# okieraised/rs-face-detection-tflite

Measured on AMD Instinct MI355X. Metric: faces/sec at batch=256 (256x256 back-camera) per GPU, higher is better.
Workload: dtype f32

## Files before the change

rs-face-detection-tflite_amd/csrc/engine.cpp:

```cpp
#include "engine.hpp"
#include "launch.hpp"

#include <algorithm>
#include <cstdio>
#include <cstdlib>
#include <cstring>
#include <stdexcept>

namespace mi {

void hip_check(hipError_t e, const char* what) {
    if (e != hipSuccess) throw std::runtime_error(std::string(what) + ": " + hipGetErrorString(e));
}

namespace {
template <class T>
void upload(T*& dev, std::vector<T>& host, const char* what_alloc, const char* what_copy) {
    if (dev) hip_check(hipFree(dev), "hipFree");
    dev = nullptr;
    if (host.empty()) return;
    hip_check(hipMalloc(reinterpret_cast<void**>(&dev), host.size() * sizeof(T)), what_alloc);
    hip_check(hipMemcpy(dev, host.data(), host.size() * sizeof(T), hipMemcpyHostToDevice), what_copy);
    std::vector<T>().swap(host);
}
// ... 53 lines not shown

const Model::Option* Model::find_option(const std::string& key) {
    using O = Option;
    constexpr int kMax = 0x7fffffff;
    static const Option table[] = {
        {"chunk", &Model::chunk_, 0, kMax, 0},
        {"graph", &Model::use_graph_, 0, 1, 0},
        {"fuse", &Model::fuse_level_, 0, 5, O::kReplan},
        {"res_budget", &Model::res_budget_, 16, 156, O::kReplan | O::kKiB},
        {"pipe", &Model::pipe_max_, 0, 4, O::kReplan},
        {"small_chain", &Model::small_chain_, 0, 64, O::kFreeSmall},
        {"pipe_rows", &Model::pipe_rows_, 1 << 1 | 1 << 2 | 1 << 4, 0, O::kOneOf},
        {"pipe_band", &Model::pipe_band_, 0, 4096, 0},
        {"strip", &Model::strip_, 0, 1, 0},
        {"stem_fuse", &Model::stem_fuse_, 0, 1, 0},
        {"stem_mfma", &Model::stem_mfma_, 0, 2, O::kForms},
        {"conv_mfma", &Model::conv_mfma_, 0, 1, 0},
        {"conv_bf16", &Model::conv_bf16_, 0, 2, O::kReplan},
        {"stem_run", &Model::stem_run_, 0, 32, 0},
        {"pair_fuse", &Model::pair_fuse_, 0, 1, 0},
        {"mdb_band", &Model::mdb_band_, 0, 4096, 0},
        {"chain_fixed", &Model::chain_fixed_, 0, 1, 0},
        {"chain_sched", &Model::chain_sched_, 0, 1, 0},
        {"mchain", &Model::mchain_, 0, 1, 0},
        {"tail", &Model::tail_, 0, 1, O::kReplan},
        {"tail_pre", &Model::tail_pre_, 0, 2, 0},
        {"tail_g", &Model::tail_g_, 0, 64, 0},
        {"band", &Model::band_, 0, 2, O::kReplan},
        {"band_test_fail", &Model::band_test_fail_, 0, 1, O::kWriteOnly},
        {"band_test_absent", &Model::band_test_absent_, 0, 256, O::kWriteOnly},
        {"band_test_gen", nullptr, 0, kMax, O::kBandGen | O::kWriteOnly},
        {"band_wide", &Model::band_wide_ok_, 0, 1, O::kReplan},
        {"band_fork", &Model::band_fork_, 0, 1, O::kReplan},
        {"band_nw", &Model::band_nw_, 8, 256, O::kReplan},
        {"band_fail_streak", &Model::band_fail_streak_, 0, 0, O::kReadOnly},
        {"band_wraps", &Model::band_wraps_, 0, 0, O::kReadOnly},
        {"fork", &Model::fork_, 0, 1, 0},
        {"heads", &Model::head_streams_opt_, 1, kHeadStreams, O::kReplan},
        {"reuse", &Model::reuse_, 0, 1, O::kReplan},
        {"lanes", &Model::lanes_, 1, 4, 0},
        {"test_poison", &Model::test_poison_, 1 << 1 | 1 << 2, 0, O::kOneOf | O::kKeepGraphs},
    };
    for (const Option& o : table)
        if (key == o.key) return &o;
    return nullptr;
}

void Model::set_option(const std::string& key, int value) {
    const Option* o = find_option(key);
    if (!o || (o->flags & Option::kReadOnly)) throw std::runtime_error("unknown option '" + key + "'");
    int v = (o->lo == 0 && o->hi == 1) ? value != 0 : std::min(o->hi, std::max(o->lo, value));
    if (o->flags & Option::kOneOf) v = (value >= 0 && value < 31 && (o->lo >> value & 1)) ? value : 0;
    if (o->flags & Option::kForms) v = (value >= o->lo && value <= o->hi) ? value : 1;
    if (o->flags & Option::kKiB) v *= 1024;
    if (o->flags & Option::kBandGen) { band_gen_ = static_cast<unsigned>(v); band_gen_force_ = true; }
    else this->*o->field = v;
    if (o->flags & Option::kKeepGraphs) return;
    if (o->flags & Option::kReplan) dirty_ = true;
    if ((o->flags & Option::kFreeSmall) && d_small_) { hipFree(d_small_); d_small_ = nullptr; small_floats_ = 0; }
    invalidate_graphs();
    chunk_cap_ = 0;
}

int Model::get_option(const std::string& key) const {
    const Option* o = find_option(key);
    if (!o || (o->flags & Option::kWriteOnly)) throw std::runtime_error("unknown option '" + key + "'");
    const int v = this->*o->field;
    return (o->flags & Option::kKiB) ? v / 1024 : v;
}

void Model::rebuild() {
    if (d_small_) { hipFree(d_small_); d_small_ = nullptr; small_floats_ = 0; }
    hip_check(hipSetDevice(device_), "hipSetDevice");
    invalidate_graphs();
    plan_ = build_plan(parse_tflite(blob_.data(), blob_.size()), fuse_level_, pipe_max_, res_budget_, tail_ != 0);
    if (!reuse_) {
        long off = 0;
        for (size_t t = 0; t < plan_.graph.tensors.size(); t++)
            if (plan_.root_offset[t] >= 0) { plan_.root_offset[t] = off; off += plan_.root_elems[t]; }
// ... 154 lines not shown
        st.bytes += bytes;
        st.macs += macs;
        auto dims = [](const std::vector<int>& sh) {
            std::string d;
            for (size_t q = 1; q < sh.size(); q++) d += (q > 1 ? "x" : "") + std::to_string(sh[q]);
            return d;
        };
        if (static_cast<int>(i) == first.launches[k].node) st.detail = dims(si) + "->";
        st.detail = st.detail.substr(0, st.detail.find("->") + 2) + dims(so);
    }
    return stats;
}

LaunchCtx Model::launch_ctx(const float* in, int chunk_start, int frames) const {
    LaunchCtx c;
    c.weights = d_weights_;
    c.arena = d_arena_ + static_cast<size_t>(plan_.arena_floats_per_frame) * chunk_cap_ * arena_lane_;
    c.in = in; c.out = d_out_.data();
    c.small = d_small_; c.small_floats = small_floats_;
    c.progs = d_programs_; c.tail_progs = d_tail_programs_;
    c.band_prog = d_band_prog_; c.band_consts = d_band_consts_; c.band_ws = d_band_ws_; c.band_sync = d_band_sync_; c.band_fail = d_band_fail_;
    c.chunk_cap = chunk_cap_; c.chunk_start = chunk_start; c.F = frames;
    c.u8_frames = u8_.frames; c.u8_lut = u8_.lut; c.u8_frame_bytes = u8_.frame_bytes; c.u8_row_bytes = u8_.row_bytes;
    c.strip = strip_; c.pair_fuse = pair_fuse_; c.stem_fuse = stem_fuse_; c.stem_mfma = stem_mfma_; c.stem_run = stem_run_; c.mchain = mchain_; c.conv_mfma = conv_mfma_; c.conv_bf16 = conv_bf16_;
    c.small_chain = small_chain_; c.lanes = lanes_;
    c.pipe_rows = pipe_rows_; c.pipe_band = pipe_band_; c.mdb_band = mdb_band_; c.tail_pre = tail_pre_; c.tail_g = tail_g_;
    c.fork = fork_ && lanes_ == 1;
    c.cu_count = device_cu_count();
    c.band = band_use_ && chunk_start == 0;
    c.band_test_absent = band_test_absent_;
    return c;
}

namespace {
int issue(const Launch& l, hipStream_t s, int chain_fixed, int chain_sched) {
    auto many = [&](int (*f)(const BlockArgs*, int, void*)) { return f(l.blocks.data(), static_cast<int>(l.blocks.size()), s); };
    switch (l.to) {
        case Launcher::Conv: return launch_conv(std::get<ConvArgs>(l.args), s);
        case Launcher::HeadGemm: return launch_head_gemm(std::get<HeadGemmArgs>(l.args), s);
        case Launcher::Dw: return launch_dw(std::get<DwArgs>(l.args), s);
        case Launcher::Xc: return launch_xc(std::get<XcArgs>(l.args), s);
        case Launcher::Mdblock: return launch_mdblock(std::get<DblockArgs>(l.args), s);
        case Launcher::Dblock: return launch_dblock(std::get<DblockArgs>(l.args), s);
        case Launcher::Mbneck: return launch_mbneck(std::get<BneckArgs>(l.args), s);
        case Launcher::Bneck: return launch_bneck(std::get<BneckArgs>(l.args), s);
        case Launcher::Tail: return launch_tail(std::get<TailLaunch>(l.args), s);
        case Launcher::Resident: return launch_resident(std::get<ResLaunch>(l.args), s);
        case Launcher::Chain: return launch_chain(std::get<ChainArgs>(l.args), s, chain_fixed, chain_sched);
        case Launcher::StripPipe: return many(launch_strip_pipe);
        case Launcher::MstripChain: return many(launch_mstrip_chain);
        case Launcher::SmallChain: {
            int rc = 0;
            for (size_t k = 0; k < l.blocks.size() && rc == 0; k++) rc = l.blocks[k].sh == 1 ? launch_strip(l.blocks[k], s) : launch_block(l.blocks[k], s);
            return rc;
        }
        case Launcher::Ms2: return launch_ms2(std::get<BlockArgs>(l.args), s);
        case Launcher::Mwalk: return launch_mwalk(std::get<BlockArgs>(l.args), s);
        case Launcher::Strip: return launch_strip(std::get<BlockArgs>(l.args), s);
        case Launcher::Mstrip: return launch_mstrip(std::get<BlockArgs>(l.args), s);
        case Launcher::Block: return launch_block(std::get<BlockArgs>(l.args), s);
        case Launcher::Add: return launch_add(std::get<EltArgs>(l.args), s);
        case Launcher::Act: return launch_act(std::get<EltArgs>(l.args), s);
        case Launcher::Maxpool: return launch_maxpool(std::get<EltArgs>(l.args), s);
        case Launcher::Padc: return launch_padc(std::get<EltArgs>(l.args), s);
        case Launcher::Resize2x: return launch_resize2x(std::get<EltArgs>(l.args), s);
        case Launcher::DepthToSpace: return launch_depth_to_space(std::get<EltArgs>(l.args), s);
        case Launcher::Bandnet: return launch_bandnet(std::get<BandLaunch>(l.args), s);
        case Launcher::Avgpool: return launch_avgpool(std::get<EltArgs>(l.args), s);
        case Launcher::L2norm: return launch_l2norm_rows(std::get<EltArgs>(l.args), s);
        case Launcher::Transpose: return launch_transpose(std::get<EltArgs>(l.args), s);
    }
    return 0;
}
// ... 228 lines not shown
            in_stage_floats_ = need;
        }
        hip_check(hipMemcpyAsync(d_in_stage_, in, need * sizeof(float), hipMemcpyHostToDevice, s), "H2D input");
        if (test_poison_ && in_stage_floats_ > need)
            hip_check(hipMemsetAsync(d_in_stage_ + need, test_poison_ == 1 ? 0xFF : 0x7F, (in_stage_floats_ - need) * sizeof(float), s), "hipMemsetAsync poison stage");
        din = d_in_stage_;
    }
    run_device(din, batch, s);
    for (int k = 0; k < num_outputs(); k++) {
        if (!outs[k]) continue;
        hip_check(hipMemcpyAsync(outs[k], d_out_[k], output_elems(k) * sizeof(float) * batch,
                                 mem == 0 ? hipMemcpyDeviceToHost : hipMemcpyDeviceToDevice, s), "copy outputs");
    }
    if (mem == 0 || !stream) hip_check(hipStreamSynchronize(s), "hipStreamSynchronize");
}

size_t Model::debug_tensor(int tensor, int frame, float* dst, size_t cap) {
    const Graph& g = plan_.graph;
    if (tensor < 0 || tensor >= static_cast<int>(g.tensors.size())) throw std::runtime_error("tensor index out of range");
    if (frame < 0 || frame >= last_chunk_frames_) throw std::runtime_error("frame outside the last chunk");
    bool produced = false;
    for (const Node& n : plan_.nodes) produced |= (n.out == tensor);
    if (!produced) throw std::runtime_error("tensor was fused away (or is an input/constant)");
    long fs;
    float* p = tensor_ptr_mut(plan_, launch_ctx(nullptr, 0, last_chunk_frames_), tensor, &fs);
    size_t n = std::min(cap, g.tensors[tensor].elems());
    hip_check(hipDeviceSynchronize(), "sync");
    hip_check(hipMemcpy(dst, p + static_cast<long>(frame) * fs, n * sizeof(float), hipMemcpyDeviceToHost), "D2H debug");
    return n;
}

}
```

rs-face-detection-tflite_amd/csrc/engine.hpp:

```cpp
#pragma once

#include <hip/hip_runtime.h>

#include <map>
#include <memory>
#include <string>
#include <vector>

#include "bandplan.hpp"
#include "consts.hpp"
#include "launches.hpp"
#include "plan.hpp"

namespace mi {

void hip_check(hipError_t e, const char* what);

class Model {
   public:
    Model(const uint8_t* bytes, size_t n, int device);
    ~Model();
    Model(const Model&) = delete;
    Model& operator=(const Model&) = delete;

// ... 30 lines not shown
    struct Option;
    static const Option* find_option(const std::string& key);
    void build_bandnet();
    void free_bandnet();
    bool band_usable(int batch) const;
    void band_before_launch(hipStream_t s);
    void poison_scratch(hipStream_t s);
    void ensure_capacity(int batch);
    LaunchCtx launch_ctx(const float* in, int chunk_start, int frames) const;
    void enqueue_chunk(const float* in, int chunk_start, int frames, hipStream_t s, std::vector<hipEvent_t>* marks = nullptr, Lowered* keep = nullptr);
    void enqueue_all(const float* in, int batch, hipStream_t s);
    void invalidate_graphs();

    int device_ = 0;
    std::vector<uint8_t> blob_;
    Plan plan_;
    int fuse_level_ = 5, pipe_max_ = 4, tail_ = 1, reuse_ = 1;
    int res_budget_ = 156 * 1024;
    int chunk_ = 0, lanes_ = 1, use_graph_ = 1;
    int fork_ = 1, head_streams_opt_ = 1;
    int conv_mfma_ = 1;
    int conv_bf16_ = 0;
    int strip_ = 1, stem_fuse_ = 1, stem_mfma_ = 1, stem_run_ = 0, pair_fuse_ = 1, mchain_ = 1, chain_fixed_ = 1, chain_sched_ = 1;
    int pipe_rows_ = 0, pipe_band_ = 0, mdb_band_ = 0;
    int tail_pre_ = 0, tail_g_ = 0;
    int arena_lane_ = 0;
    std::vector<hipStream_t> side_streams_;
    std::vector<hipEvent_t> lane_events_;
    SideSchedule sched_;
    std::vector<hipStream_t> head_streams_;
    std::vector<hipEvent_t> head_events_;
    bool dirty_ = true;

    float* d_weights_ = nullptr;
    PlanConsts consts_;
    int profile_inner_ = 1;

    ResStage* d_programs_ = nullptr;
    TailStage* d_tail_programs_ = nullptr;
    float* d_arena_ = nullptr;
    size_t arena_floats_ = 0;
    int chunk_cap_ = 0;
    int batch_cap_ = 0;
    std::vector<float*> d_out_;
    float* d_in_stage_ = nullptr;
    size_t in_stage_floats_ = 0;
// ... 54 lines not shown
```

rs-face-detection-tflite_amd/csrc/kernels.hpp:

```cpp
#pragma once

#include <cstddef>
#include <cstdint>

namespace mi {

enum ActKind : int { ACT_NONE = 0, ACT_RELU = 1, ACT_RELU6 = 2, ACT_PRELU = 3 };
enum ResMode : int { RES_NONE = 0, RES_DIRECT = 1, RES_MAXPOOL = 2, RES_UP2X = 3 };

struct Epilogue {
    const float* bias = nullptr;
    const float* alpha = nullptr;
    const float* res = nullptr;
    long res_fs = 0;
    int res_mode = RES_NONE;
    int res_C = 0;
    int res_W = 0, res_H = 0;
    int act = ACT_NONE;
    int res_after = 0;
};

struct ConvArgs {
    const float* in = nullptr;
    const uint8_t* in_u8 = nullptr;
// ... 254 lines not shown
int strip_consts_floats(int C);
void strip_pack_consts(int C, const float* w_dw, const float* b_dw, const float* w_pw, const float* bias, const float* alpha, int act, float* dst);
const char* strip_kernel_label(const BlockArgs& a, char* buf, size_t cap);
int launch_mwalk(const BlockArgs& a, void* stream);
bool mwalk_kernel_supports(const BlockArgs& a);
bool mwalk_shape_ok(int W, int C, int Co);
int mwalk_consts_floats(int W, int C, int Co);
void mwalk_pack_consts(int W, int C, int Co, const float* w_dw, const float* b_dw, const float* w_pw, const float* bias, const float* alpha, int act, float* dst);
const char* mwalk_kernel_label(const BlockArgs& a, char* buf, size_t cap);
int launch_ms2(const BlockArgs& a, void* stream);
bool ms2_kernel_supports(const BlockArgs& a);
bool ms2_shape_ok(int W, int C, int Co, bool skip);
int ms2_consts_floats(int W, int C, int Co, bool skip);
void ms2_pack_consts(int W, int C, int Co, bool skip, const float* w_dw, const float* b_dw, const float* w_pw, const float* bias, const float* alpha, int act, float* dst);
const char* ms2_kernel_label(const BlockArgs& a, char* buf, size_t cap);
int launch_mstrip(const BlockArgs& a, void* stream);
bool mstrip_kernel_supports(const BlockArgs& a);
bool mstrip_shape_ok(int C, int Co);
int mstrip_consts_floats(int C);
void mstrip_pack_consts(int C, const float* w_dw, const float* b_dw, const float* w_pw, const float* bias, const float* alpha, int act, float* dst);
const char* mstrip_kernel_label(const BlockArgs& a, char* buf, size_t cap);
bool mstrip_chain_supports(const BlockArgs* blocks, int n);
int launch_mstrip_chain(const BlockArgs* blocks, int n, void* stream);
bool strip_pipe_supports(const BlockArgs* blocks, int n);
bool strip_pipe_shape_ok(int C, int W);
bool strip_tail_shape_ok(int C, int Co, int H, int W);
int strip_consts_s2_floats(int C, int Co);
void strip_pack_consts_s2(int C, int Co, const float* w_dw, const float* b_dw, const float* w_pw, const float* bias, const float* alpha, int act, float* dst);
int launch_strip_pipe(const BlockArgs* blocks, int n, void* stream);
const char* strip_pipe_label(const BlockArgs* blocks, int n, char* buf, size_t cap);
int strip_pipe_rows_per_step(int H, int hint = 0);
int launch_chain(const ChainArgs& a, void* stream, int fixed = 1, int sched = 1);

struct BneckBlock {
    const float* w1 = nullptr;
    const float* w2 = nullptr;
    const float* consts = nullptr;
    float hi1 = 0.f, hi2 = 0.f;
    const float* mconsts = nullptr;
    int act1 = ACT_RELU, act2 = ACT_RELU;
};
constexpr int kMaxBneck = 6;
struct BneckArgs {
    const float* in = nullptr;
    float* out = nullptr;
    long in_fs = 0, out_fs = 0;
// ... 163 lines not shown
```

rs-face-detection-tflite_amd/csrc/launches.cpp:

```cpp
#include "launches.hpp"

#include <algorithm>
#include <cmath>
#include <cstdio>
#include <cstdlib>
#include <stdexcept>

namespace mi {

namespace {
void same_pad(int in, int k, int stride, int out, int* before) { *before = std::max(0, (out - 1) * stride + k - in) / 2; }
bool is_view(const Node& n) { return n.kind == Node::Reshape || n.kind == Node::Concat; }
int dim(const std::vector<int>& v, size_t d) { return d < v.size() ? v[d] : 1; }
float clamp_of(int act) { return act == ACT_RELU6 ? 6.f : INFINITY; }
}

bool band_cut(const BandPlan& bp, size_t i) { return static_cast<int>(i) >= bp.first && !bp.node_runs[i]; }

int band_run_launches(const Plan& plan, const BandPlan& bp) {
    int launches = 1;
    for (size_t i = 0; i < plan.nodes.size(); i++)
        if (!is_view(plan.nodes[i]) && !band_cut(bp, i)) launches++;
    return launches;
}
// ... 519 lines not shown
                if (b.ep.res_mode != RES_NONE) { b.ep.res = cur; b.ep.res_fs = cur_fs; }
                if (k == nb - 1) { b.out = op; b.out_fs = out_fs; } else { b.out = T[k & 1]; b.out_fs = fsz; }
                ok = b.sh == 1 ? strip_kernel_supports(b) : block_kernel_supports(b);
                cur = b.out; cur_fs = b.out_fs;
            }
            if (ok) {
                l.to = Launcher::SmallChain;
                if (want_labels) {
                    char name[48];
                    const bool s2 = sb[static_cast<size_t>(nb - 1)].sh == 2;
                    snprintf(buf, sizeof buf, "%s x%d%s (small batch)", strip_kernel_label(sb[0], name, sizeof name), s2 ? nb - 1 : nb, s2 ? " + block_kernel" : "");
                    l.label = buf;
                }
                l.blocks = std::move(sb);
                return;
            }
        }
        if (!strip_pipe_supports(blk.data(), static_cast<int>(blk.size()))) throw std::runtime_error("chain node without a kernel");
        l.to = Launcher::StripPipe;
        if (want_labels) l.label = strip_pipe_label(blk.data(), static_cast<int>(blk.size()), buf, sizeof buf);
        l.blocks = std::move(blk);
    }

    size_t block(size_t i, Launch& l) const {
        const Node& n = plan.nodes[i];
        const BlockArgs a = block_args(i);
        char buf[96];
        if (c.strip && c.pair_fuse && pc.node_pair[i] >= 0 && i + 1 < plan.nodes.size() && !sched.event_after[i] && sched.slot[i + 1] < 0 && sched.slot[i] < 0) {
            const Node& nb = plan.nodes[i + 1];
            const DblockArgs d = dblock_args(a.in, a.in_fs, n.in[0], nb.out, n, nb, pc.node_pair[i], true);
            const bool apart = d.out + d.out_fs * c.F <= d.in || d.in + d.in_fs * c.F <= d.out;
            if (apart && mdblock_kernel_supports(d)) {
                set(l, Launcher::Mdblock, d, lab("mdblock_kernel<pair>"));
                return 2;
            }
        }
        if (c.strip && ms2_kernel_supports(a)) {
            set(l, Launcher::Ms2, a, want_labels ? ms2_kernel_label(a, buf, sizeof buf) : nullptr);
            return 1;
        }
        if (c.strip && mwalk_kernel_supports(a)) {
            set(l, Launcher::Mwalk, a, want_labels ? mwalk_kernel_label(a, buf, sizeof buf) : nullptr);
            return 1;
        }
        const bool strip = c.strip && strip_kernel_supports(a);
        const bool mstrip = c.strip && !strip && mstrip_kernel_supports(a);
        if (mstrip && c.mchain && c.lanes == 1) {
            std::vector<BlockArgs> run{a};
            for (size_t j = i + 1; j < plan.nodes.size() && run.size() < 8; j++) {
                const Node& m = plan.nodes[j];
                if (m.kind != Node::Block || m.w < 0 || m.in.size() != 1 || m.in[0] != plan.nodes[j - 1].out || pc.node_strip[j] < 0 || sched.slot[j] >= 0) break;
                if (shape(m.in[0]).size() != 4 || shape(m.out) != shape(m.in[0]) || m.ept >= 0) break;
                if (m.res >= 0 && (m.res != m.in[0] || m.res_mode != RES_DIRECT || m.res_after)) break;
                run.push_back(block_args(j));
                if (!mstrip_chain_supports(run.data(), static_cast<int>(run.size()))) { run.pop_back(); break; }
            }
            if (run.size() >= 2) {
                l.to = Launcher::MstripChain;
                if (want_labels) { snprintf(buf, sizeof buf, "mstrip_chain_kernel<%d,%d>", a.C / 4, a.ep.act == ACT_RELU ? 1 : 0); l.label = buf; }
                l.blocks = std::move(run);
                return l.blocks.size();
            }
        }
        if (strip) set(l, Launcher::Strip, a, want_labels ? strip_kernel_label(a, buf, sizeof buf) : nullptr);
        else if (mstrip) set(l, Launcher::Mstrip, a, want_labels ? mstrip_kernel_label(a, buf, sizeof buf) : nullptr);
        else set(l, Launcher::Block, a, want_labels ? block_kernel_label(a, buf, sizeof buf) : nullptr);
        return 1;
    }
};

}

Lowered lower_chunk(const Plan& plan, const PlanConsts& consts, const BandPlan& bp, const SideSchedule& sched, const LaunchCtx& c, bool want_labels) {
    const Lowering lo{plan, consts, bp, sched, c, want_labels};
    const size_t N = plan.nodes.size();
    Lowered out;
// ... 37 lines not shown
```

rs-face-detection-tflite_amd/csrc/launches.hpp:

```cpp
#pragma once

#include <string>
#include <variant>
#include <vector>

#include "bandplan.hpp"
#include "consts.hpp"
#include "kernels.hpp"
#include "plan.hpp"

namespace mi {

constexpr int kHeadStreams = 4;

struct SideSchedule {
    std::vector<int> slot, wait;
    std::vector<char> event_after;
};
SideSchedule schedule_side_streams(const Plan& plan, int head_streams);

struct LaunchCtx {
    const float* weights = nullptr;
    float* arena = nullptr;
    const float* in = nullptr;
    float* const* out = nullptr;
    float* small = nullptr;
    size_t small_floats = 0;
    const ResStage* progs = nullptr;
    const TailStage* tail_progs = nullptr;
    const BandPacked* band_prog = nullptr;
    const float* band_consts = nullptr;
    float* band_ws = nullptr;
    unsigned* band_sync = nullptr;
    int* band_fail = nullptr;
    int chunk_cap = 0, chunk_start = 0, F = 0;
    const uint8_t* u8_frames = nullptr;
    const float* u8_lut = nullptr;
    long u8_frame_bytes = 0;
    int u8_row_bytes = 0;
    int strip = 1, pair_fuse = 1, stem_fuse = 1, stem_mfma = 1, stem_run = 0, mchain = 1, small_chain = 16, lanes = 1;
    int conv_mfma = 1;
    int conv_bf16 = 0;
    int pipe_rows = 0, pipe_band = 0, mdb_band = 0, tail_pre = 0, tail_g = 0;
    bool fork = true;
    int cu_count = 256;
    bool band = false;
    int band_test_absent = 0;
};

enum class Launcher {
    Conv, HeadGemm, Dw, Xc, Mdblock, Dblock, Mbneck, Bneck, Tail, Resident, Chain, StripPipe, SmallChain, Ms2, Mwalk, MstripChain, Strip, Mstrip, Block,
    Add, Act, Maxpool, Padc, Resize2x, DepthToSpace, Bandnet, Avgpool, L2norm, Transpose
};

struct Launch {
    Launcher to = Launcher::Conv;
    std::variant<ConvArgs, HeadGemmArgs, DwArgs, XcArgs, DblockArgs, BneckArgs, TailLaunch, ResLaunch, ChainArgs, BlockArgs, EltArgs, BandLaunch> args;
    std::vector<BlockArgs> blocks;
    int node = -1, last = -1;
    int slot = -1;
    int wait = -1;
    bool record = false;
    std::string label;
};

struct Lowered {
    std::vector<Launch> launches;
    std::vector<int> launch_of_node;
};
Lowered lower_chunk(const Plan& plan, const PlanConsts& consts, const BandPlan& band_plan, const SideSchedule& sched, const LaunchCtx& ctx, bool want_labels);

float* tensor_ptr_mut(const Plan& plan, const LaunchCtx& ctx, int t, long* frame_stride);

bool band_cut(const BandPlan& band_plan, size_t i);
int band_run_launches(const Plan& plan, const BandPlan& band_plan);
// ... 5 lines not shown
```

rs-face-detection-tflite_amd/csrc/mrow.hpp:

```cpp
#pragma once

#include <hip/hip_runtime.h>

#include <type_traits>
#include <utility>

#include "kernels.hpp"
#include "launch.hpp"
#include "wave_sync.hpp"

namespace mi {

namespace {

typedef float df32x4 __attribute__((ext_vector_type(4)));

__device__ __forceinline__ void dwg_barrier() {
    asm volatile("s_waitcnt lgkmcnt(0)\n\ts_barrier" ::: "memory");
}

template <class F, int... KS>
__device__ __forceinline__ void dfor_each(F&& f, std::integer_sequence<int, KS...>) { (f(std::integral_constant<int, KS>{}), ...); }

typedef float dv2f __attribute__((ext_vector_type(2)));
// ... 102 lines not shown
            aC[ks].s[0] = c;
            aPN[ks].s[0] = n;
            asm volatile("" : "+v"(aC[ks].s[0]), "+v"(aPN[ks].s[0]));
            pch[nt] = pc;
        }
        if constexpr (EMIT) {
            if constexpr (NP > 0) __builtin_amdgcn_sched_barrier(0);
#pragma unroll
            for (int mt = 0; mt < MT; mt++)
#pragma unroll
                for (int nt = 0; nt < WT; nt++) D[mt][nt] = __builtin_amdgcn_mfma_f32_16x16x4f32(aw[mt], pch[nt], D[mt][nt], 0, 0, 0);
        }
        asm volatile("s_waitcnt lgkmcnt(0)" ::: "memory");
        if constexpr (ks + 1 < CK) landed(xs[(ks + 1) & 1], av[(ks + 1) & 1]);
        __builtin_amdgcn_sched_barrier(0);
    };
    load_ks(std::integral_constant<int, 0>{}, xs[0], av[0]);
    asm volatile("s_waitcnt lgkmcnt(0)" ::: "memory");
    landed(xs[0], av[0]);
    __builtin_amdgcn_sched_barrier(0);
    dfor_each(kstep, std::make_integer_sequence<int, CK>{});
}

template <int CK, int MT, int PS, bool EMIT>
__device__ __forceinline__ void mstrip_row(const unsigned xr, const unsigned ar, const float (&tap)[CK][9], float (&aPN)[CK][2], float (&aC)[CK][2], df32x4 (&D)[MT][2]) {
    float xs[2][3][2], av[2][MT];
    auto load_ks = [&](auto ksc, float (&x)[3][2], float (&aw)[MT]) {
        constexpr int ks = decltype(ksc)::value;
        const unsigned xa = xr, aa = ar;
#pragma unroll
        for (int dx = 0; dx < 3; dx++) {
            asm volatile("ds_read_b32 %0, %1 offset:%2" : "=v"(x[dx][0]) : "v"(xa), "n"((dx * PS + 4 * ks) * 4));
            asm volatile("ds_read_b32 %0, %1 offset:%2" : "=v"(x[dx][1]) : "v"(xa), "n"((dx * PS + 4 * ks + 16 * PS) * 4));
        }
        if constexpr (EMIT) {
#pragma unroll
            for (int mt = 0; mt < MT; mt++) asm volatile("ds_read_b32 %0, %1 offset:%2" : "=v"(aw[mt]) : "v"(aa), "n"((ks * MT + mt) * 64 * 4));
        }
    };
    auto landed = [&](float (&x)[3][2], float (&aw)[MT]) {
#pragma unroll
        for (int dx = 0; dx < 3; dx++) asm volatile("" : "+v"(x[dx][0]), "+v"(x[dx][1]));
        if constexpr (EMIT) {
#pragma unroll
            for (int mt = 0; mt < MT; mt++) asm volatile("" : "+v"(aw[mt]));
        }
    };
    auto kstep = [&](auto ksc) {
        constexpr int ks = decltype(ksc)::value;
        if constexpr (ks + 1 < CK) load_ks(std::integral_constant<int, ks + 1>{}, xs[(ks + 1) & 1], av[(ks + 1) & 1]);
        float (&x)[3][2] = xs[ks & 1];
        float (&aw)[MT] = av[ks & 1];
        const float (&w)[9] = tap[ks];
        float pch[2];
#pragma unroll
        for (int nt = 0; nt < 2; nt++) {
            float n = x[0][nt] * w[0], c = aC[ks][nt], pc = aPN[ks][nt];
#pragma unroll
            for (int dx = 0; dx < 3; dx++) {
                if (EMIT) pc = __builtin_fmaf(x[dx][nt], w[6 + dx], pc);
                if (dx) n = __builtin_fmaf(x[dx][nt], w[dx], n);
                c = __builtin_fmaf(x[dx][nt], w[3 + dx], c);
            }
            aC[ks][nt] = c;
            aPN[ks][nt] = n;
            asm volatile("" : "+v"(aC[ks][nt]), "+v"(aPN[ks][nt]));
            pch[nt] = pc;
        }
        if constexpr (EMIT) {
#pragma unroll
            for (int mt = 0; mt < MT; mt++) {
                D[mt][0] = __builtin_amdgcn_mfma_f32_16x16x4f32(aw[mt], pch[0], D[mt][0], 0, 0, 0);
                D[mt][1] = __builtin_amdgcn_mfma_f32_16x16x4f32(aw[mt], pch[1], D[mt][1], 0, 0, 0);
            }
        }
        asm volatile("s_waitcnt lgkmcnt(0)" ::: "memory");
        if constexpr (ks + 1 < CK) landed(xs[(ks + 1) & 1], av[(ks + 1) & 1]);
        __builtin_amdgcn_sched_barrier(0);
    };
    load_ks(std::integral_constant<int, 0>{}, xs[0], av[0]);
    asm volatile("s_waitcnt lgkmcnt(0)" ::: "memory");
    landed(xs[0], av[0]);
    __builtin_amdgcn_sched_barrier(0);
    dfor_each(kstep, std::make_integer_sequence<int, CK>{});
}


typedef __attribute__((address_space(1))) char gchar;
typedef __attribute__((address_space(1))) df32x4 gf32x4;

template <int CK>
__device__ __forceinline__ int mrow_goff(int lane) { return ((lane / (CK + 1)) * 4 * CK + 4 * min(lane % (CK + 1), CK - 1)) * 4; }

constexpr unsigned mrow_exec_hi(int active) { return active == 64 ? 0xffffffffu : (1u << (active - 32)) - 1; }

template <int C, int PS, int DPX, int ACTIVE>
__device__ __forceinline__ void mrow_dma2(const char* src, const unsigned dstb, const int goff) {
// ... 179 lines not shown
```

rs-face-detection-tflite_amd/csrc/mstrip_kernels.hip:

```cpp
#include <hip/hip_runtime.h>

#include <algorithm>
#include <cstdint>
#include <cstdio>
#include <cstdlib>
#include <type_traits>
#include <utility>

#include "kernels.hpp"
#include "launch.hpp"
#include "mrow.hpp"

namespace mi {

namespace {

struct MstripArgs {
    const float* in;
    float* out;
    const float* consts;
    long in_fs, out_fs;
    int B, H;
    int bands, band_rows;
    int has_res;
// ... 39 lines not shown
__device__ __forceinline__ void mstrip_issue_row(const float* in, const int r, const int H, const unsigned lds_img, const int bi, const int goff) {
    using K = MK<CK>;
    mrow_dma2<K::C, K::PS, K::DPX, K::DPX * K::QP>(reinterpret_cast<const char*>(in + (long)min(max(r, 0), H - 1) * 32 * K::C),
                                                   lds_img + (unsigned)((bi * K::IMG_F + K::PS) * 4), goff);
}

template <int CK, bool RELU, class HR>
__device__ __forceinline__ void mstrip_walk(const float* in, float* out, const float* wgc, float* img, const unsigned lds_img, const int goff, const HR has_res,
                                            const float hi, const int H, const int y0, const int y1, const int lane, MstripStamps& st) {
    using K = MK<CK>;
    constexpr int C = K::C, MT = K::MT, PS = K::PS, QP = K::QP, IMG_F = K::IMG_F, NLD = K::NLD;
    const int kq = lane >> 4, p = lane & 15;
    float tap[CK][9];
    mrow_load_taps9<CK>(reinterpret_cast<const float4*>(wgc + K::A_F + 2 * C) + kq * 3, tap);
    MI_MSTAMP(0)
    typedef __attribute__((address_space(3))) float lfloat;
    const unsigned x_lds = (unsigned)(uintptr_t)(lfloat*)(img + p * PS + kq);
    const unsigned a_lds = (unsigned)(uintptr_t)(lfloat*)const_cast<float*>(wgc + lane);
    const float* sme = img + (1 + p) * PS + 4 * kq;
    const unsigned ooff = (unsigned)(p * C + 4 * kq) * 4u;

    float accA[CK][2], accB[CK][2];
    df32x4 D[MT][2];
#pragma unroll
    for (int ks = 0; ks < CK; ks++) accA[ks][0] = accA[ks][1] = accB[ks][0] = accB[ks][1] = 0.f;

    constexpr int NST = 2 * MT;
    auto step = [&](auto emit, int r, float (&aPN)[CK][2], float (&aC)[CK][2]) {
        const int t = r - (y0 - 1), bi = t & 1;
        mrow_wait<NST, NLD>(t - 1 >= 2, t == 0 || (t - 1) + 2 <= (y1 - y0 + 1));
        if (r < 0 || r >= H) mrow_clear_row<32 * QP>(img + bi * IMG_F + PS, lane);
        wave_sync();
        MI_MSTAMP(1)
        mstrip_row<CK, MT, PS, decltype(emit)::value>(x_lds + (unsigned)(bi * IMG_F * 4), a_lds, tap, aPN, aC, D);
        MI_MSTAMP(2)
        __builtin_amdgcn_sched_barrier(0);
        if constexpr (decltype(emit)::value) mrow_store_row<RELU, C, 32>(D, (gchar*)(out + (long)(r - 1) * 32 * C), ooff, wgc + K::A_F + C + 4 * kq, hi, p);
        MI_MSTAMP(3)
        __builtin_amdgcn_sched_barrier(0);
        mrow_init_acc<C, PS>(D, wgc + K::A_F + 4 * kq, sme + bi * IMG_F, has_res != 0);
        __builtin_amdgcn_sched_barrier(0);
        wave_sync();
        __builtin_amdgcn_s_waitcnt(0xC07F);
        if (r + 2 <= y1) mstrip_issue_row<CK>(in, r + 2, H, lds_img, bi, goff);
        MI_MSTAMP(4)
    };
    step(std::false_type{}, y0 - 1, accA, accB);
    step(std::false_type{}, y0, accB, accA);
    for (int r = y0 + 1; r <= y1; r += 2) {
        step(std::true_type{}, r, accA, accB);
        if (r + 1 > y1) break;
        step(std::true_type{}, r + 1, accB, accA);
    }
}

template <int CK, bool RELU>
__global__ __launch_bounds__(256, 2) void mstrip_kernel(MstripArgs a) {
// ... 73 lines not shown
        mstrip_issue_row<CK>(in, y0, ca.H, lds_img, 1, goff);
        wait_vm<NLD>();
        asm volatile("s_waitcnt lgkmcnt(0)" ::: "memory");
        if (blk == 0) {
            __builtin_amdgcn_s_barrier();
            asm volatile("" ::: "memory");
        }
        mstrip_walk<CK, RELU>(in, outp, wgc, img, lds_img, goff, has_res, hi, ca.H, y0, y1, lane, st);
        asm volatile("s_waitcnt vmcnt(0)" ::: "memory");
        if (more) {
            float* nx = lds + ((blk + 1) & 1) * K::WG_F;
#pragma unroll
            for (int k = 0; k < NPRE; k++) {
                const int i = threadIdx.x + 512 * k;
                if (i < K::WG_F / 4) reinterpret_cast<float4*>(nx)[i] = pre[k];
            }
        }
        asm volatile("s_waitcnt vmcnt(0) lgkmcnt(0)" ::: "memory");
        __builtin_amdgcn_s_barrier();
        asm volatile("" ::: "memory");
    }
}

}

bool mstrip_shape_ok(int C, int Co) {
    static const bool off = getenv("MI_NO_MSTRIP") != nullptr;
    return !off && C == Co && C == 48;
}

bool mstrip_kernel_supports(const BlockArgs& a) {
    if (!a.w_strip || !a.has_dw || a.sh != 1 || a.sw != 1 || a.pt != 1 || a.pl != 1) return false;
    if (!mstrip_shape_ok(a.C, a.Co) || a.W != 32 || a.H != a.Ho || a.W != a.Wo || a.H < 2) return false;
    if (a.ep.res_mode != RES_NONE) {
        if (a.ep.res_after) return false;
        if (a.ep.res_mode != RES_DIRECT || a.ep.res != a.in || a.ep.res_fs != a.in_fs || a.ep.res_C != a.C) return false;
    }
    static const int min_b = getenv("MI_MSTRIP_MIN_B") ? atoi(getenv("MI_MSTRIP_MIN_B")) : 32;
    if (a.B < min_b) return false;
    return aligned16(a.in) && aligned16(a.out) && !(a.in_fs & 3) && !(a.out_fs & 3);
}

int mstrip_consts_floats(int C) { return C == 48 ? MK<12>::TOTAL : 0; }

void mstrip_pack_consts(int C, const float* w_dw, const float* b_dw, const float* w_pw, const float* bias, const float* alpha, int act, float* dst) {
    using K = MK<12>;
    std::fill(dst, dst + mstrip_consts_floats(C), 0.f);
    mrow_pack_a(dst + K::OFF_A, w_pw, C / 4, K::MT, C);
    mrow_pack_taps(dst + K::OFF_TAP, w_dw, C / 4);
    mrow_pack_bias(dst + K::OFF_BIAS, dst + K::OFF_SLOPE, C, C, w_pw, b_dw, bias, alpha, act);
}

const char* mstrip_kernel_label(const BlockArgs& a, char* buf, size_t cap) {
    snprintf(buf, cap, "mstrip_kernel<%d,%d>", a.C / 4, a.ep.act == ACT_RELU ? 1 : 0);
    return buf;
}

bool mstrip_chain_supports(const BlockArgs* blocks, int n) {
    static const bool off = getenv("MI_NO_MSTRIP_CHAIN") != nullptr;
    if (off || n < 2 || n > kMstripChain) return false;
    for (int k = 0; k < n; k++) {
        const BlockArgs& a = blocks[k];
        if (!mstrip_kernel_supports(a) || a.H != 32 || a.B != blocks[0].B || (a.ep.act == ACT_RELU) != (blocks[0].ep.act == ACT_RELU)) return false;
        if (k && a.in != blocks[k - 1].out) return false;
    }
    return true;
}

int launch_mstrip_chain(const BlockArgs* blocks, int n, void* stream) {
    using K = MK<12>;
    if (!mstrip_chain_supports(blocks, n)) return (int)hipErrorInvalidValue;
    MstripChainArgs ca{};
    ca.nblocks = n; ca.B = blocks[0].B; ca.H = blocks[0].H;
    for (int k = 0; k < n; k++) {
        const BlockArgs& a = blocks[k];
        ca.in[k] = a.in; ca.out[k] = a.out; ca.consts[k] = a.w_strip; ca.in_fs[k] = a.in_fs; ca.out_fs[k] = a.out_fs;
        ca.has_res[k] = a.ep.res_mode == RES_DIRECT;
        ca.hi[k] = a.ep.act == ACT_RELU6 ? 6.f : INFINITY;
    }
    const size_t lds_bytes = (size_t)(2 * K::WG_F + 8 * K::NBUF * K::IMG_F) * 4;
    return mrow_launch(mstrip_chain_kernel<12, true>, mstrip_chain_kernel<12, false>, blocks[0].ep.act == ACT_RELU, dim3((unsigned)ca.B), dim3(512), lds_bytes,
                       (hipStream_t)stream, ca);
}

unsigned long long* g_mstrip_stamps = nullptr;

int launch_mstrip(const BlockArgs& a, void* stream) {
    using K = MK<12>;
    MstripArgs ma;
    ma.stamps = g_mstrip_stamps;
    ma.in = a.in; ma.out = a.out; ma.consts = a.w_strip; ma.in_fs = a.in_fs; ma.out_fs = a.out_fs;
    ma.B = a.B; ma.H = a.H;
    static const int forced = getenv("MI_MSTRIP_BAND") ? atoi(getenv("MI_MSTRIP_BAND")) : 0;
    long bands = std::max<long>(1, (8L * device_cu_count() + a.B / 2) / std::max(1, a.B));
    int rows = (int)((a.H + bands - 1) / bands);
    rows = std::max(rows, std::min(a.H, 4));
    if (forced > 0) rows = std::min(forced, a.H);
    ma.band_rows = rows;
    ma.bands = (a.H + rows - 1) / rows;
    ma.has_res = a.ep.res_mode == RES_DIRECT;
    ma.hi = a.ep.act == ACT_RELU6 ? 6.f : INFINITY;
    const long units = (long)a.B * ma.bands;
    const size_t lds_bytes = (size_t)(K::WG_F + 4 * K::NBUF * K::IMG_F) * 4;
    return mrow_launch(mstrip_kernel<12, true>, mstrip_kernel<12, false>, a.ep.act == ACT_RELU, dim3((unsigned)((units + 3) / 4)), dim3(256), lds_bytes,
                       (hipStream_t)stream, ma);
// ... 4 lines not shown
```

Before: 224,100.

## Add row-pipelined mstrip kernel fusing consecutive C=48 blocks through LDS rings

Adds a new mstrip_pipe kernel that fuses 2-4 consecutive depthwise+pointwise C=48, 32x32 blocks into one launch. Each pair of waves owns one block, and rows stream from one block to the next through LDS ring buffers, so intermediate activations never go to global memory. The pointwise weights stay in registers rather than being re-read from LDS. It is enabled by default when the chunk has at least 256 frames, and the debug tensor readback now rejects tensors fused away this way. The cost is higher register pressure and fewer frames per workgroup (one per block), which may reduce occupancy compared with the existing mstrip chain kernel.

Result: no change. 224,700, median of 6 (+0.3%).

```diff
diff --git a/rs-face-detection-tflite_amd/csrc/engine.cpp b/rs-face-detection-tflite_amd/csrc/engine.cpp
--- a/rs-face-detection-tflite_amd/csrc/engine.cpp
+++ b/rs-face-detection-tflite_amd/csrc/engine.cpp
@@ -99,7 +99,7 @@
         {"mdb_band", &Model::mdb_band_, 0, 4096, 0},
         {"chain_fixed", &Model::chain_fixed_, 0, 1, 0},
         {"chain_sched", &Model::chain_sched_, 0, 1, 0},
-        {"mchain", &Model::mchain_, 0, 1, 0},
+        {"mchain", &Model::mchain_, 0, 2, O::kForms},
         {"tail", &Model::tail_, 0, 1, O::kReplan},
         {"tail_pre", &Model::tail_pre_, 0, 2, 0},
         {"tail_g", &Model::tail_g_, 0, 64, 0},
@@ -132,6 +132,7 @@
     if (o->flags & Option::kKiB) v *= 1024;
     if (o->flags & Option::kBandGen) { band_gen_ = static_cast<unsigned>(v); band_gen_force_ = true; }
     else this->*o->field = v;
+    if (o->field == &Model::mchain_) mchain_set_ = true;
     if (o->flags & Option::kKeepGraphs) return;
     if (o->flags & Option::kReplan) dirty_ = true;
     if ((o->flags & Option::kFreeSmall) && d_small_) { hipFree(d_small_); d_small_ = nullptr; small_floats_ = 0; }
@@ -332,7 +333,7 @@
     c.band_prog = d_band_prog_; c.band_consts = d_band_consts_; c.band_ws = d_band_ws_; c.band_sync = d_band_sync_; c.band_fail = d_band_fail_;
     c.chunk_cap = chunk_cap_; c.chunk_start = chunk_start; c.F = frames;
     c.u8_frames = u8_.frames; c.u8_lut = u8_.lut; c.u8_frame_bytes = u8_.frame_bytes; c.u8_row_bytes = u8_.row_bytes;
-    c.strip = strip_; c.pair_fuse = pair_fuse_; c.stem_fuse = stem_fuse_; c.stem_mfma = stem_mfma_; c.stem_run = stem_run_; c.mchain = mchain_; c.conv_mfma = conv_mfma_; c.conv_bf16 = conv_bf16_;
+    c.strip = strip_; c.pair_fuse = pair_fuse_; c.stem_fuse = stem_fuse_; c.stem_mfma = stem_mfma_; c.stem_run = stem_run_; c.mchain = mchain_; c.mpipe_from = mchain_set_ ? 0 : kMstripPipeMinFrames; c.conv_mfma = conv_mfma_; c.conv_bf16 = conv_bf16_;
     c.small_chain = small_chain_; c.lanes = lanes_;
     c.pipe_rows = pipe_rows_; c.pipe_band = pipe_band_; c.mdb_band = mdb_band_; c.tail_pre = tail_pre_; c.tail_g = tail_g_;
     c.fork = fork_ && lanes_ == 1;
@@ -359,6 +360,7 @@
         case Launcher::Chain: return launch_chain(std::get<ChainArgs>(l.args), s, chain_fixed, chain_sched);
         case Launcher::StripPipe: return many(launch_strip_pipe);
         case Launcher::MstripChain: return many(launch_mstrip_chain);
+        case Launcher::MstripPipe: return many(launch_mstrip_pipe);
         case Launcher::SmallChain: {
             int rc = 0;
             for (size_t k = 0; k < l.blocks.size() && rc == 0; k++) rc = l.blocks[k].sh == 1 ? launch_strip(l.blocks[k], s) : launch_block(l.blocks[k], s);
@@ -633,8 +635,12 @@
     bool produced = false;
     for (const Node& n : plan_.nodes) produced |= (n.out == tensor);
     if (!produced) throw std::runtime_error("tensor was fused away (or is an input/constant)");
+    const LaunchCtx ctx = launch_ctx(nullptr, 0, last_chunk_frames_);
+    for (const Launch& l : lower_chunk(plan_, consts_, band_plan_, sched_, ctx, false).launches)
+        for (int i = l.node; l.to == Launcher::MstripPipe && i < l.last; i++)
+            if (plan_.nodes[static_cast<size_t>(i)].out == tensor) throw std::runtime_error("tensor was fused away (or is an input/constant)");
     long fs;
-    float* p = tensor_ptr_mut(plan_, launch_ctx(nullptr, 0, last_chunk_frames_), tensor, &fs);
+    float* p = tensor_ptr_mut(plan_, ctx, tensor, &fs);
     size_t n = std::min(cap, g.tensors[tensor].elems());
     hip_check(hipDeviceSynchronize(), "sync");
     hip_check(hipMemcpy(dst, p + static_cast<long>(frame) * fs, n * sizeof(float), hipMemcpyDeviceToHost), "D2H debug");
diff --git a/rs-face-detection-tflite_amd/csrc/engine.hpp b/rs-face-detection-tflite_amd/csrc/engine.hpp
--- a/rs-face-detection-tflite_amd/csrc/engine.hpp
+++ b/rs-face-detection-tflite_amd/csrc/engine.hpp
@@ -76,6 +76,7 @@
     int conv_mfma_ = 1;
     int conv_bf16_ = 0;
     int strip_ = 1, stem_fuse_ = 1, stem_mfma_ = 1, stem_run_ = 0, pair_fuse_ = 1, mchain_ = 1, chain_fixed_ = 1, chain_sched_ = 1;
+    bool mchain_set_ = false;
     int pipe_rows_ = 0, pipe_band_ = 0, mdb_band_ = 0;
     int tail_pre_ = 0, tail_g_ = 0;
     int arena_lane_ = 0;
diff --git a/rs-face-detection-tflite_amd/csrc/kernels.hpp b/rs-face-detection-tflite_amd/csrc/kernels.hpp
--- a/rs-face-detection-tflite_amd/csrc/kernels.hpp
+++ b/rs-face-detection-tflite_amd/csrc/kernels.hpp
@@ -300,6 +300,11 @@
 const char* mstrip_kernel_label(const BlockArgs& a, char* buf, size_t cap);
 bool mstrip_chain_supports(const BlockArgs* blocks, int n);
 int launch_mstrip_chain(const BlockArgs* blocks, int n, void* stream);
+bool mstrip_block_ok(const BlockArgs& a);
+bool mstrip_pipe_supports(const BlockArgs* blocks, int n);
+int launch_mstrip_pipe(const BlockArgs* blocks, int n, void* stream);
+const char* mstrip_pipe_label(const BlockArgs* blocks, int n, char* buf, size_t cap);
+constexpr int kMstripPipeMinFrames = 256;
 bool strip_pipe_supports(const BlockArgs* blocks, int n);
 bool strip_pipe_shape_ok(int C, int W);
 bool strip_tail_shape_ok(int C, int Co, int H, int W);
diff --git a/rs-face-detection-tflite_amd/csrc/launches.cpp b/rs-face-detection-tflite_amd/csrc/launches.cpp
--- a/rs-face-detection-tflite_amd/csrc/launches.cpp
+++ b/rs-face-detection-tflite_amd/csrc/launches.cpp
@@ -565,6 +565,25 @@
         l.blocks = std::move(blk);
     }
 
+    bool mstrip_run_member(size_t j) const {
+        const Node& m = plan.nodes[j];
+        if (m.kind != Node::Block || m.w < 0 || m.in.size() != 1 || m.in[0] != plan.nodes[j - 1].out || pc.node_strip[j] < 0 || sched.slot[j] >= 0) return false;
+        if (shape(m.in[0]).size() != 4 || shape(m.out) != shape(m.in[0]) || m.ept >= 0) return false;
+        return !(m.res >= 0 && (m.res != m.in[0] || m.res_mode != RES_DIRECT || m.res_after));
+    }
+    bool feeds_only_next(size_t j) const {
+        const int t = plan.nodes[j - 1].out;
+        if (sched.event_after[j - 1]) return false;
+        for (int o : g.outputs)
+            if (plan.storage[o].root == plan.storage[t].root) return false;
+        for (size_t k = 0; k < plan.nodes.size(); k++) {
+            if (k == j) continue;
+            const Node& m = plan.nodes[k];
+            if (m.res == t || std::find(m.in.begin(), m.in.end(), t) != m.in.end()) return false;
+        }
+        return true;
+    }
+
     size_t block(size_t i, Launch& l) const {
         const Node& n = plan.nodes[i];
         const BlockArgs a = block_args(i);
@@ -588,13 +607,22 @@
         }
         const bool strip = c.strip && strip_kernel_supports(a);
         const bool mstrip = c.strip && !strip && mstrip_kernel_supports(a);
+        const bool mpipe = c.mchain == 2 || (c.mchain == 1 && c.mpipe_from > 0 && c.F >= c.mpipe_from);
+        if (c.strip && !strip && mpipe && c.lanes == 1 && mstrip_block_ok(a)) {
+            std::vector<BlockArgs> run{a};
+            for (size_t j = i + 1; j < plan.nodes.size() && run.size() < 8 && mstrip_run_member(j) && feeds_only_next(j); j++) run.push_back(block_args(j));
+            for (size_t n = run.size() <= 4 ? run.size() : std::min<size_t>(4, run.size() - 2); n >= 2; n--) {
+                if (!mstrip_pipe_supports(run.data(), static_cast<int>(n))) continue;
+                run.resize(n);
+                l.to = Launcher::MstripPipe;
+                if (want_labels) l.label = mstrip_pipe_label(run.data(), static_cast<int>(n), buf, sizeof buf);
+                l.blocks = std::move(run);
+                return n;
+            }
+        }
         if (mstrip && c.mchain && c.lanes == 1) {
             std::vector<BlockArgs> run{a};
-            for (size_t j = i + 1; j < plan.nodes.size() && run.size() < 8; j++) {
-                const Node& m = plan.nodes[j];
-                if (m.kind != Node::Block || m.w < 0 || m.in.size() != 1 || m.in[0] != plan.nodes[j - 1].out || pc.node_strip[j] < 0 || sched.slot[j] >= 0) break;
-                if (shape(m.in[0]).size() != 4 || shape(m.out) != shape(m.in[0]) || m.ept >= 0) break;
-                if (m.res >= 0 && (m.res != m.in[0] || m.res_mode != RES_DIRECT || m.res_after)) break;
+            for (size_t j = i + 1; j < plan.nodes.size() && run.size() < 8 && mstrip_run_member(j); j++) {
                 run.push_back(block_args(j));
                 if (!mstrip_chain_supports(run.data(), static_cast<int>(run.size()))) { run.pop_back(); break; }
             }
diff --git a/rs-face-detection-tflite_amd/csrc/launches.hpp b/rs-face-detection-tflite_amd/csrc/launches.hpp
--- a/rs-face-detection-tflite_amd/csrc/launches.hpp
+++ b/rs-face-detection-tflite_amd/csrc/launches.hpp
@@ -39,6 +39,7 @@
     long u8_frame_bytes = 0;
     int u8_row_bytes = 0;
     int strip = 1, pair_fuse = 1, stem_fuse = 1, stem_mfma = 1, stem_run = 0, mchain = 1, small_chain = 16, lanes = 1;
+    int mpipe_from = kMstripPipeMinFrames;
     int conv_mfma = 1;
     int conv_bf16 = 0;
     int pipe_rows = 0, pipe_band = 0, mdb_band = 0, tail_pre = 0, tail_g = 0;
@@ -50,7 +51,7 @@
 
 enum class Launcher {
     Conv, HeadGemm, Dw, Xc, Mdblock, Dblock, Mbneck, Bneck, Tail, Resident, Chain, StripPipe, SmallChain, Ms2, Mwalk, MstripChain, Strip, Mstrip, Block,
-    Add, Act, Maxpool, Padc, Resize2x, DepthToSpace, Bandnet, Avgpool, L2norm, Transpose
+    Add, Act, Maxpool, Padc, Resize2x, DepthToSpace, Bandnet, Avgpool, L2norm, Transpose, MstripPipe
 };
 
 struct Launch {
diff --git a/rs-face-detection-tflite_amd/csrc/mrow.hpp b/rs-face-detection-tflite_amd/csrc/mrow.hpp
--- a/rs-face-detection-tflite_amd/csrc/mrow.hpp
+++ b/rs-face-detection-tflite_amd/csrc/mrow.hpp
@@ -148,26 +148,32 @@
     dfor_each(kstep, std::make_integer_sequence<int, CK>{});
 }
 
-template <int CK, int MT, int PS, bool EMIT>
-__device__ __forceinline__ void mstrip_row(const unsigned xr, const unsigned ar, const float (&tap)[CK][9], float (&aPN)[CK][2], float (&aC)[CK][2], df32x4 (&D)[MT][2]) {
-    float xs[2][3][2], av[2][MT];
-    auto load_ks = [&](auto ksc, float (&x)[3][2], float (&aw)[MT]) {
+template <int CK, int MT, int PS, bool EMIT, int WT = 2, bool AREG = false>
+__device__ __forceinline__ void mstrip_row(const unsigned xr, const unsigned ar, const float (&tap)[CK][9], float (&aPN)[CK][WT], float (&aC)[CK][WT], df32x4 (&D)[MT][WT],
+                                           const float (&areg)[AREG ? CK : 1][MT]) {
+    static_assert(WT == 1 || WT == 2, "one or two pixel tiles");
+    constexpr bool ALDS = EMIT && !AREG;
+    float xs[2][3][WT], av[2][MT];
+    auto load_ks = [&](auto ksc, float (&x)[3][WT], float (&aw)[MT]) {
         constexpr int ks = decltype(ksc)::value;
         const unsigned xa = xr, aa = ar;
 #pragma unroll
         for (int dx = 0; dx < 3; dx++) {
             asm volatile("ds_read_b32 %0, %1 offset:%2" : "=v"(x[dx][0]) : "v"(xa), "n"((dx * PS + 4 * ks) * 4));
-            asm volatile("ds_read_b32 %0, %1 offset:%2" : "=v"(x[dx][1]) : "v"(xa), "n"((dx * PS + 4 * ks + 16 * PS) * 4));
-        }
-        if constexpr (EMIT) {
+            if constexpr (WT == 2) asm volatile("ds_read_b32 %0, %1 offset:%2" : "=v"(x[dx][WT - 1]) : "v"(xa), "n"((dx * PS + 4 * ks + 16 * PS) * 4));
+        }
+        if constexpr (ALDS) {
 #pragma unroll
             for (int mt = 0; mt < MT; mt++) asm volatile("ds_read_b32 %0, %1 offset:%2" : "=v"(aw[mt]) : "v"(aa), "n"((ks * MT + mt) * 64 * 4));
         }
     };
-    auto landed = [&](float (&x)[3][2], float (&aw)[MT]) {
-#pragma unroll
-        for (int dx = 0; dx < 3; dx++) asm volatile("" : "+v"(x[dx][0]), "+v"(x[dx][1]));
-        if constexpr (EMIT) {
+    auto landed = [&](float (&x)[3][WT], float (&aw)[MT]) {
+#pragma unroll
+        for (int dx = 0; dx < 3; dx++) {
+            if constexpr (WT == 2) asm volatile("" : "+v"(x[dx][0]), "+v"(x[dx][WT - 1]));
+            else asm volatile("" : "+v"(x[dx][0]));
+        }
+        if constexpr (ALDS) {
 #pragma unroll
             for (int mt = 0; mt < MT; mt++) asm volatile("" : "+v"(aw[mt]));
         }
@@ -175,12 +181,12 @@
     auto kstep = [&](auto ksc) {
         constexpr int ks = decltype(ksc)::value;
         if constexpr (ks + 1 < CK) load_ks(std::integral_constant<int, ks + 1>{}, xs[(ks + 1) & 1], av[(ks + 1) & 1]);
-        float (&x)[3][2] = xs[ks & 1];
-        float (&aw)[MT] = av[ks & 1];
+        float (&x)[3][WT] = xs[ks & 1];
+        const float* const aw = AREG ? areg[AREG ? ks : 0] : av[ks & 1];
         const float (&w)[9] = tap[ks];
-        float pch[2];
-#pragma unroll
-        for (int nt = 0; nt < 2; nt++) {
+        float pch[WT];
+#pragma unroll
+        for (int nt = 0; nt < WT; nt++) {
             float n = x[0][nt] * w[0], c = aC[ks][nt], pc = aPN[ks][nt];
 #pragma unroll
             for (int dx = 0; dx < 3; dx++) {
@@ -195,10 +201,9 @@
         }
         if constexpr (EMIT) {
 #pragma unroll
-            for (int mt = 0; mt < MT; mt++) {
-                D[mt][0] = __builtin_amdgcn_mfma_f32_16x16x4f32(aw[mt], pch[0], D[mt][0], 0, 0, 0);
-                D[mt][1] = __builtin_amdgcn_mfma_f32_16x16x4f32(aw[mt], pch[1], D[mt][1], 0, 0, 0);
-            }
+            for (int mt = 0; mt < MT; mt++)
+#pragma unroll
+                for (int nt = 0; nt < WT; nt++) D[mt][nt] = __builtin_amdgcn_mfma_f32_16x16x4f32(aw[mt], pch[nt], D[mt][nt], 0, 0, 0);
         }
         asm volatile("s_waitcnt lgkmcnt(0)" ::: "memory");
         if constexpr (ks + 1 < CK) landed(xs[(ks + 1) & 1], av[(ks + 1) & 1]);
diff --git a/rs-face-detection-tflite_amd/csrc/mstrip_kernels.hip b/rs-face-detection-tflite_amd/csrc/mstrip_kernels.hip
--- a/rs-face-detection-tflite_amd/csrc/mstrip_kernels.hip
+++ b/rs-face-detection-tflite_amd/csrc/mstrip_kernels.hip
@@ -85,6 +85,7 @@
 
     float accA[CK][2], accB[CK][2];
     df32x4 D[MT][2];
+    const float no_areg[1][MT] = {};
 #pragma unroll
     for (int ks = 0; ks < CK; ks++) accA[ks][0] = accA[ks][1] = accB[ks][0] = accB[ks][1] = 0.f;
 
@@ -95,7 +96,7 @@
         if (r < 0 || r >= H) mrow_clear_row<32 * QP>(img + bi * IMG_F + PS, lane);
         wave_sync();
         MI_MSTAMP(1)
-        mstrip_row<CK, MT, PS, decltype(emit)::value>(x_lds + (unsigned)(bi * IMG_F * 4), a_lds, tap, aPN, aC, D);
+        mstrip_row<CK, MT, PS, decltype(emit)::value>(x_lds + (unsigned)(bi * IMG_F * 4), a_lds, tap, aPN, aC, D, no_areg);
         MI_MSTAMP(2)
         __builtin_amdgcn_sched_barrier(0);
         if constexpr (decltype(emit)::value) mrow_store_row<RELU, C, 32>(D, (gchar*)(out + (long)(r - 1) * 32 * C), ooff, wgc + K::A_F + C + 4 * kq, hi, p);
@@ -215,6 +216,101 @@
     }
 }
 
+constexpr int kMstripPipe = 4;
+struct MstripPipeArgs {
+    const float* in;
+    float* out;
+    const float* consts[kMstripPipe];
+    long in_fs, out_fs;
+    int has_res[kMstripPipe];
+    float hi[kMstripPipe];
+    int B, H;
+};
+
+template <int CK, int KB>
+struct MP {
+    using K = MK<CK>;
+    static constexpr int NIN = 3, NRING = 2 * (KB - 1);
+    static constexpr int OFF_ZERO = KB * 2 * K::C, OFF_IN = OFF_ZERO + K::IMG_F, OFF_RING = OFF_IN + NIN * K::IMG_F, TOTAL = OFF_RING + NRING * K::IMG_F;
+    static_assert(TOTAL * 4 <= kLdsBudget, "LDS");
+};
+
+template <int CK, int KB, bool RELU>
+__global__ __launch_bounds__(128 * KB, 2) void mstrip_pipe_kernel(MstripPipeArgs a) {
+    using K = MK<CK>;
+    using P = MP<CK, KB>;
+    constexpr int C = K::C, MT = K::MT, PS = K::PS, QP = K::QP, IMG_F = K::IMG_F;
+    extern __shared__ __attribute__((aligned(16))) float lds[];
+    typedef __attribute__((address_space(3))) float lfloat;
+    const int lane = threadIdx.x & 63;
+    const int wave = __builtin_amdgcn_readfirstlane(threadIdx.x >> 6);
+    const int j = wave >> 1, h = wave & 1;
+    const int kq = lane >> 4, p = lane & 15;
+    const int H = a.H;
+    const float* in = a.in + (long)blockIdx.x * a.in_fs;
+    float* out = a.out + (long)blockIdx.x * a.out_fs;
+    const float* cj = a.consts[j];
+    const int goff = mrow_goff<CK>(lane);
+    const unsigned lds0 = __builtin_amdgcn_readfirstlane((unsigned)(uintptr_t)(lfloat*)lds);
+    auto issue = [&](const int r) {
+        mrow_dma1<4, C, PS, K::DPX, K::DPX * QP>(reinterpret_cast<const char*>(in + ((long)r * 32 + 16 * h) * C),
+                                                 lds0 + (unsigned)((P::OFF_IN + ((r + 1) % 3) * IMG_F + (1 + 16 * h) * PS) * 4), goff);
+    };
+    if (j == 0) issue(0);
+    for (int i = threadIdx.x; i < IMG_F / 4; i += 128 * KB) reinterpret_cast<float4*>(lds + P::OFF_ZERO)[i] = make_float4(0.f, 0.f, 0.f, 0.f);
+    if (wave == 2 * KB - 1) mrow_clear_border<QP, P::NIN + P::NRING, IMG_F, 33 * PS>(lds + P::OFF_IN, lane);
+    for (int i = 64 * h + lane; i < 2 * C; i += 128) lds[j * 2 * C + i] = cj[K::OFF_BIAS + i];
+    float tap[CK][9], areg[CK][MT];
+    mrow_load_taps9<CK>(reinterpret_cast<const float4*>(cj + K::OFF_TAP) + kq * 3, tap);
+#pragma unroll
+    for (int ks = 0; ks < CK; ks++)
+#pragma unroll
+        for (int mt = 0; mt < MT; mt++) areg[ks][mt] = cj[K::OFF_A + (ks * MT + mt) * 64 + lane];
+#pragma unroll
+    for (int ks = 0; ks < CK; ks++)
+#pragma unroll
+        for (int mt = 0; mt < MT; mt++) asm volatile("" : "+v"(areg[ks][mt]));
+    const unsigned x_off = (unsigned)(((16 * h + p) * PS + kq) * 4);
+    const int d_off = (1 + 16 * h + p) * PS + 4 * kq;
+    const unsigned ooff = (unsigned)(((16 * h + p) * C + 4 * kq) * 4);
+    const float* bias = lds + j * 2 * C + 4 * kq;
+    const int has_res = a.has_res[j];
+    const float hi = a.hi[j];
+
+    float accA[CK][1], accB[CK][1];
+    df32x4 D[MT][1];
+#pragma unroll
+    for (int ks = 0; ks < CK; ks++) accA[ks][0] = accB[ks][0] = 0.f;
+    dwg_barrier();
+
+    auto step = [&](auto emit, const int t, const int r, float (&aPN)[CK][1], float (&aC)[CK][1]) {
+        const int src = r < 0 || r >= H ? P::OFF_ZERO : (j == 0 ? P::OFF_IN + (t % 3) * IMG_F : P::OFF_RING + (2 * (j - 1) + ((t + 1) & 1)) * IMG_F);
+        mstrip_row<CK, MT, PS, decltype(emit)::value, 1, true>(lds0 + (unsigned)(src * 4) + x_off, 0u, tap, aPN, aC, D, areg);
+        __builtin_amdgcn_sched_barrier(0);
+        if constexpr (decltype(emit)::value) {
+            if (j == KB - 1) mrow_store_row<RELU, C, 32>(D, (gchar*)(out + (long)(r - 1) * 32 * C), ooff, bias + C, hi, p);
+            else mrow_store_a<RELU, C, PS>(D, lds + P::OFF_RING + (2 * j + (t & 1)) * IMG_F + d_off, bias + C, hi, true, kq);
+        }
+        __builtin_amdgcn_sched_barrier(0);
+        mrow_init_acc<C, PS>(D, bias, lds + src + d_off, has_res != 0);
+        __builtin_amdgcn_sched_barrier(0);
+    };
+    auto phase = [&](const int t, float (&aPN)[CK][1], float (&aC)[CK][1]) {
+        const int r = t - 1 - 2 * j;
+        if (j == 0 && t + 1 < H) issue(t + 1);
+        if (r >= 1 && r <= H) step(std::true_type{}, t, r, aPN, aC);
+        else if (r >= -1 && r <= 0) step(std::false_type{}, t, r, aPN, aC);
+        if (j == 0) {
+            if (t + 1 < H) wait_vm<4>(); else wait_vm<0>();
+        }
+        dwg_barrier();
+    };
+    for (int t = 0; t < H + 2 * KB; t += 2) {
+        phase(t, accA, accB);
+        phase(t + 1, accB, accA);
+    }
+}
+
 }
 
 bool mstrip_shape_ok(int C, int Co) {
@@ -222,16 +318,20 @@
     return !off && C == Co && C == 48;
 }
 
-bool mstrip_kernel_supports(const BlockArgs& a) {
+bool mstrip_block_ok(const BlockArgs& a) {
     if (!a.w_strip || !a.has_dw || a.sh != 1 || a.sw != 1 || a.pt != 1 || a.pl != 1) return false;
     if (!mstrip_shape_ok(a.C, a.Co) || a.W != 32 || a.H != a.Ho || a.W != a.Wo || a.H < 2) return false;
     if (a.ep.res_mode != RES_NONE) {
         if (a.ep.res_after) return false;
         if (a.ep.res_mode != RES_DIRECT || a.ep.res != a.in || a.ep.res_fs != a.in_fs || a.ep.res_C != a.C) return false;
     }
+    return aligned16(a.in) && aligned16(a.out) && !(a.in_fs & 3) && !(a.out_fs & 3);
+}
+
+bool mstrip_kernel_supports(const BlockArgs& a) {
+    if (!mstrip_block_ok(a)) return false;
     static const int min_b = getenv("MI_MSTRIP_MIN_B") ? atoi(getenv("MI_MSTRIP_MIN_B")) : 32;
-    if (a.B < min_b) return false;
-    return aligned16(a.in) && aligned16(a.out) && !(a.in_fs & 3) && !(a.out_fs & 3);
+    return a.B >= min_b;
 }
 
 int mstrip_consts_floats(int C) { return C == 48 ? MK<12>::TOTAL : 0; }
@@ -274,6 +374,45 @@
     const size_t lds_bytes = (size_t)(2 * K::WG_F + 8 * K::NBUF * K::IMG_F) * 4;
     return mrow_launch(mstrip_chain_kernel<12, true>, mstrip_chain_kernel<12, false>, blocks[0].ep.act == ACT_RELU, dim3((unsigned)ca.B), dim3(512), lds_bytes,
                        (hipStream_t)stream, ca);
+}
+
+bool mstrip_pipe_supports(const BlockArgs* blocks, int n) {
+    if (n < 2 || n > kMstripPipe) return false;
+    for (int k = 0; k < n; k++) {
+        const BlockArgs& a = blocks[k];
+        if (!mstrip_block_ok(a) || a.H != 32 || a.B != blocks[0].B || a.B < 1 || (a.ep.act == ACT_RELU) != (blocks[0].ep.act == ACT_RELU)) return false;
+        if (k && a.in != blocks[k - 1].out) return false;
+    }
+    const BlockArgs &f = blocks[0], &l = blocks[n - 1];
+    const bool apart = l.out + l.out_fs * l.B <= f.in || f.in + f.in_fs * f.B <= l.out;
+    return apart || (l.out == f.in && l.out_fs == f.in_fs);
+}
+
+const char* mstrip_pipe_label(const BlockArgs* blocks, int n, char* buf, size_t cap) {
+    snprintf(buf, cap, "mstrip_pipe_kernel<%d,%d,%d>", blocks[0].C / 4, n, blocks[0].ep.act == ACT_RELU ? 1 : 0);
+    return buf;
+}
+
+namespace {
+template <int KB>
+int launch_mstrip_pipe_kb(const MstripPipeArgs& pa, bool relu, hipStream_t stream) {
+    return mrow_launch(mstrip_pipe_kernel<12, KB, true>, mstrip_pipe_kernel<12, KB, false>, relu, dim3((unsigned)pa.B), dim3(128 * KB), (size_t)MP<12, KB>::TOTAL * 4, stream, pa);
+}
+}
+
+int launch_mstrip_pipe(const BlockArgs* blocks, int n, void* stream) {
+    if (!mstrip_pipe_supports(blocks, n)) return (int)hipErrorInvalidValue;
+    MstripPipeArgs pa{};
+    pa.in = blocks[0].in; pa.in_fs = blocks[0].in_fs; pa.out = blocks[n - 1].out; pa.out_fs = blocks[n - 1].out_fs;
+    pa.B = blocks[0].B; pa.H = blocks[0].H;
+    for (int k = 0; k < kMstripPipe; k++) {
+        const BlockArgs& a = blocks[std::min(k, n - 1)];
+        pa.consts[k] = a.w_strip;
+        pa.has_res[k] = a.ep.res_mode == RES_DIRECT;
+        pa.hi[k] = a.ep.act == ACT_RELU6 ? 6.f : INFINITY;
+    }
+    const bool relu = blocks[0].ep.act == ACT_RELU;
+    return n == 2 ? launch_mstrip_pipe_kb<2>(pa, relu, (hipStream_t)stream) : n == 3 ? launch_mstrip_pipe_kb<3>(pa, relu, (hipStream_t)stream) : launch_mstrip_pipe_kb<4>(pa, relu, (hipStream_t)stream);
 }
 
 unsigned long long* g_mstrip_stamps = nullptr;
```
